# LeonOrou/OPF-Graph-Neural-Solver

Hardware: AMD Instinct MI355X
Metric: grids/sec (fwd+bwd) on batched case118, K=4 (higher is better)
Workload: dtype f32

## Files before the change

opf-graph-neural-solver_amd/csrc/gns_api.hip:

```cpp
#include <atomic>
#include <cmath>
#include <cstring>
#include <cstdlib>
#include <mutex>
#include "gns_kernels.h"
#include "gns_gridwg.h"

namespace {
struct GnsTuning {
  int fwd_mapping;
  int gw_pack;
  int fwd_waves;
  int fwd_plane;
  int dw_mfma;
  int train_mapping;
  int bwd_variant;
  int team;
  int bwds_mode;
  int bwds_chunks;
};
GnsTuning make_tuning() {
  GnsTuning t{0, 0, GNS_FWD_THREADS / 64, 2, 1, 0, 4, 0, 1, 0};
  if (const char* e = std::getenv("GNS_TEAM")) { const int v = std::atoi(e); if (v >= 0 && v <= GNS_MAX_TEAM) t.team = v; }
  if (const char* e = std::getenv("GNS_FWD_MAPPING")) t.fwd_mapping = !std::strcmp(e, "lane") ? 1 : (!std::strcmp(e, "lds") ? 2 : 0);
// ... 351 lines not shown
  *status = word ? 1 : 0;
  return GNS_OK;
}

extern "C" int gns_prepack_bytes(const gns_config* cfg, int64_t Bt, size_t* bytes) {
  int rc = check_cfg(cfg);
  if (rc != GNS_OK) return rc;
  if (!bytes || Bt <= 0) return GNS_EINVAL;
  const int64_t groups = (Bt + GNS_LANES - 1) / GNS_LANES;
  *bytes = (size_t)groups * gns_in_rows(cfg->n_bus, cfg->n_line) * GNS_LANES * 16;
  return GNS_OK;
}

extern "C" int gns_prepack(const gns_config* cfg, const void* topo_dev, const float* buses, const float* lines,
                           const float* generators, int64_t Bt, void* packed, size_t packed_bytes, void* stream) {
  size_t need = 0;
  int rc = gns_prepack_bytes(cfg, Bt, &need);
  if (rc != GNS_OK) return rc;
  if (!topo_dev || !buses || !lines || !generators || !packed) return GNS_EINVAL;
  if (packed_bytes < need) return GNS_ESIZE;
  return gns_launch_pack_inputs((const int*)topo_dev, buses, lines, generators, (float*)packed, cfg->n_bus, cfg->n_line, cfg->n_gen, Bt,
                                (Bt + GNS_LANES - 1) / GNS_LANES, (hipStream_t)stream);
}

static int lane_forward(const gns_config* cfg, const GnsFamilies& fam, const GnsFwdLayout& L, char* ws, float* pt, float* pin,
                        const int* topo_dev, const int* group_topo, const int* slot_grid, int64_t Bt, float* v, float* theta,
                        float* total_loss, float* last_loss, int save_state, hipStream_t st) {
  const int N = cfg->n_bus, E = cfg->n_line, K = cfg->K, d = cfg->latent_dim, h = cfg->hidden_dim;
  const GnsTuning& T = tuning();
  int rc;
  GnsFwdArgs A;
  std::memset(&A, 0, sizeof(A));
  A.topo = topo_dev; A.group_topo = group_topo; A.slot_grid = slot_grid; A.pt = pt; A.in = pin;
  A.state = (float*)(ws + L.off_state); A.lam = (float*)(ws + L.off_lam); A.msg = (float*)(ws + L.off_msg);
  A.v_out = v; A.theta_out = theta; A.total_out = total_loss; A.last_out = last_loss;
  for (int i = 0; i < fam.nfam; ++i) { A.t_off[i] = fam.t_off[i]; A.t_sz[i] = fam.t_sz[i]; }
  for (int k = 0; k < K; ++k) A.gw[k] = (float)std::pow((double)cfg->gamma, (double)(K - k));
  A.Bt = Bt; A.G = L.groups; A.N = N; A.E = E; A.K = K; A.save = save_state ? 1 : 0;
  const int team0 = lane_team(L.groups * GNS_LANES);
  A.team = team0;
  A.team_ws = (unsigned char*)(ws + L.off_team);
  int waves = T.fwd_waves;
  while (waves * A.team > GNS_MAXP) waves /= 2;
  A.part_idx = gns_part_index(waves * A.team);
  auto pick_planes = [&]() {
    A.plane = (device().fwd_ready && gns_fwd_plane_fits(N, A.team) && T.fwd_plane) ? 1 : 0;
    if (A.plane && gns_fwd_plane2_fits(N, A.team) && T.fwd_plane == 2) A.plane = 2;
  };
  pick_planes();
  if (A.team > 1) {
    const int per_cu = gns_fwd_blocks_per_cu(d, h, cfg->multiple_phi, A, waves * 64);
    if ((long long)per_cu * device().ncu < A.G * A.team) {
      A.team = 1;
      waves = T.fwd_waves;
      A.part_idx = gns_part_index(waves);
      pick_planes();
    }
  }
  if (team0 > 1 && hipMemsetAsync(A.team_ws, 0, (size_t)L.groups * GNS_TEAM_CTR_BYTES, st) != hipSuccess) return GNS_ELAUNCH;
  record_forward(1, waves, A.plane, A.team, -1);
  prof_mark(0, true, st);
  rc = gns_launch_forward(d, h, cfg->multiple_phi, A, waves * 64, st);
  prof_mark(0, false, st);
  return rc;
}

static int split_backward(const gns_config* cfg, const GnsFamilies& fam, const GnsFwdLayout& L, const GnsBwdsLayout& S, const char* fw,
                          char* bw, const int* topo_dev, const int* group_topo, const int* slot_grid, const float* params,
                          const void* packed_inputs, int64_t Bt, const float* grad_total, const float* grad_last, const float* grad_v,
                          const float* grad_theta, float* grad_params, hipStream_t st, const IgradOut* ig = nullptr) {
  const int N = cfg->n_bus, E = cfg->n_line, K = cfg->K, d = cfg->latent_dim, h = cfg->hidden_dim;
  int rc;
  GnsBwdsArgs A;
  std::memset(&A, 0, sizeof(A));
  A.topo = topo_dev; A.group_topo = group_topo; A.slot_grid = slot_grid;
  A.pt = (const float*)(fw + L.off_pt); A.pn = (const float*)(fw + L.off_pn);
  A.in = packed_inputs ? (const float*)packed_inputs : (const float*)(fw + L.off_in);
  A.state = (const float*)(fw + L.off_state); A.lam = (const float*)(fw + L.off_lam); A.msg = (const float*)(fw + L.off_msg);
  A.g_total = grad_total; A.g_last = grad_last; A.g_v = grad_v; A.g_theta = grad_theta;
  A.adj = (float*)(bw + S.off_adj); A.slots = (float*)(bw + S.off_slots); A.slab = (float*)(bw + S.off_slab);
  for (int i = 0; i < fam.nfam; ++i) {
    A.t_off[i] = fam.t_off[i]; A.t_sz[i] = fam.t_sz[i]; A.n_off[i] = fam.n_off[i]; A.n_sz[i] = fam.n_sz[i];
    A.g_off[i] = fam.g_off[i]; A.g_sz[i] = fam.g_sz[i];
  }
  A.Bt = Bt; A.G = S.groups; A.slab_floats = S.slab_floats; A.N = N; A.E = E; A.K = K;
  A.C = S.C; A.part_idx = gns_part_index(S.C); A.R = S.R;
  A.RB = (int)(1 + S.mq); A.RBA = (int)S.adj_rows;
  A.mode = cfg->multiple_phi ? tuning().bwds_mode : 2;
  const size_t lds = gns_bwds_phys_lds(N, &A.use_plane);
  if (ig) {
    A.igrad = ig->buf;
    if (hipMemsetAsync(A.igrad, 0, ig->bytes, st) != hipSuccess) return GNS_ELAUNCH;
  }
  record_backward(4, 1, A.mode, A.C, A.R, -1);
  prof_mark(1, true, st);
  for (int k = K - 1; k >= 0; --k) {
    A.k = k;
    A.gwk = (float)std::pow((double)cfg->gamma, (double)(K - k));
    rc = gns_launch_bwds_phys(A, lds, st);
    if (rc != GNS_OK) return rc;
    if (ig) {
      rc = gns_launch_bwds_igrad_phys(A, st);
      if (rc != GNS_OK) return rc;
    }
    rc = gns_launch_bwds_sweep(d, h, cfg->multiple_phi, A, st);
    if (rc != GNS_OK) return rc;
  }
  if (ig && (ig->buses || ig->lines || ig->gens)) {
    rc = gns_launch_bwds_igrad_unpack(A, ig->in_buses, ig->in_lines, ig->in_gens, cfg->n_gen, ig->buses, ig->lines, ig->gens, st);
    if (rc != GNS_OK) return rc;
  }
// ... 120 lines not shown
    rc = gns_gw_launch_backward(d, h, cfg->multiple_phi, G, GL.blocks, st);
    prof_mark(1, false, st);
    if (rc != GNS_OK) return rc;
    return gns_launch_reduce(G.slab, (float*)(bw + GL.off_part), (float*)(bw + GL.off_tmp), params, grad_params, GL.nslab,
                             GL.slab_floats, fam, K, d, h, st);
  }
  GnsFwdLayout L;
  gns_fwd_layout(N, E, d, h, K, cfg->multiple_phi, Bt, 1, &L);
  if (use_split_backward(cfg)) {
    GnsBwdsLayout S;
    gns_bwds_layout(N, E, d, h, K, cfg->multiple_phi, Bt, device().ncu, tuning().bwds_chunks, &S);
    if (fwd_workspace_bytes < L.total || bwd_workspace_bytes < S.total) return GNS_ESIZE;
    GnsFamilies fam; gns_families_padded(model->latent_dim, model->hidden_dim, d, h, K, cfg->multiple_phi, &fam);
    return split_backward(cfg, fam, L, S, (const char*)fwd_workspace, (char*)bwd_workspace, (const int*)topo_dev, nullptr, nullptr, params,
                          packed_inputs, Bt, grad_total, grad_last, grad_v, grad_theta, grad_params, (hipStream_t)stream);
  }
  GnsBwdLayout B;
  const int team = lane_team(Bt);
  gns_bwd_layout(N, E, d, h, K, cfg->multiple_phi, Bt, team, &B);
  if (fwd_workspace_bytes < L.total || bwd_workspace_bytes < B.total) return GNS_ESIZE;
  GnsFamilies fam; gns_families_padded(model->latent_dim, model->hidden_dim, d, h, K, cfg->multiple_phi, &fam);
  hipStream_t st = (hipStream_t)stream;
  const char* fw = (const char*)fwd_workspace;
  char* bw = (char*)bwd_workspace;
  const int blocks = (int)(B.groups * team < GNS_BWD_MAX_WG ? B.groups * team : GNS_BWD_MAX_WG);
  const long long nslab = (long long)blocks * GNS_BWD_WAVES;
  const bool v2 = tuning().dw_mfma && tuning().bwd_variant >= 2 && cfg->multiple_phi;
  if (!v2 && hipMemsetAsync(bw + B.off_slab, 0, (size_t)nslab * B.slab_floats * 4, st) != hipSuccess) return GNS_ELAUNCH;
  GnsBwdArgs A;
  std::memset(&A, 0, sizeof(A));
  A.topo = (const int*)topo_dev;
  A.pt = (const float*)(fw + L.off_pt); A.pn = (const float*)(fw + L.off_pn);
  A.in = packed_inputs ? (const float*)packed_inputs : (const float*)(fw + L.off_in);
  A.state = (const float*)(fw + L.off_state); A.lam = (const float*)(fw + L.off_lam); A.msg = (const float*)(fw + L.off_msg);
  A.g_total = grad_total; A.g_last = grad_last; A.g_v = grad_v; A.g_theta = grad_theta;
  A.adj = (float*)(bw + B.off_adj); A.slots = (float*)(bw + B.off_slots); A.slab = (float*)(bw + B.off_slab);
  for (int i = 0; i < fam.nfam; ++i) {
    A.t_off[i] = fam.t_off[i]; A.t_sz[i] = fam.t_sz[i]; A.n_off[i] = fam.n_off[i]; A.n_sz[i] = fam.n_sz[i];
    A.g_off[i] = fam.g_off[i]; A.g_sz[i] = fam.g_sz[i];
  }
  for (int k = 0; k < K; ++k) A.gw[k] = (float)std::pow((double)cfg->gamma, (double)(K - k));
  A.Bt = Bt; A.G = B.groups; A.slab_floats = B.slab_floats; A.N = N; A.E = E; A.K = K;
  A.part_idx = gns_part_index(GNS_BWD_WAVES * team);
  A.team = team; A.team_ws = (unsigned char*)(bw + B.off_team);
  if (team > 1 && hipMemsetAsync(A.team_ws, 0, (size_t)B.groups * GNS_TEAM_CTR_BYTES, st) != hipSuccess) return GNS_ELAUNCH;
  A.slab_dirty = v2 ? 1 : 0;
  record_backward(tuning().dw_mfma && cfg->multiple_phi && (tuning().bwd_variant == 2 || tuning().bwd_variant == 3) ? tuning().bwd_variant : 1,
                  tuning().dw_mfma, -1, -1, -1, -1);
  prof_mark(1, true, st);
  rc = gns_launch_backward(d, h, cfg->multiple_phi, tuning().dw_mfma, tuning().bwd_variant, A, blocks, st);
  prof_mark(1, false, st);
  if (rc != GNS_OK) return rc;
  return gns_launch_reduce(A.slab, (float*)(bw + B.off_part), (float*)(bw + B.off_tmp), params, grad_params, blocks, B.slab_floats,
                           fam, K, d, h, st, (long long)GNS_BWD_WAVES * B.slab_floats);
}

extern "C" int gns_backward_inputs(const gns_config* cfg, const void* topo_dev, const float* params,
                                   const float* buses, const float* lines, const float* generators, int64_t Bt, const void* packed_inputs,
                                   const void* fwd_workspace, size_t fwd_workspace_bytes, const float* grad_total,
                                   const float* grad_last, const float* grad_v, const float* grad_theta, float* grad_params,
                                   float* grad_buses, float* grad_lines, float* grad_generators,
                                   void* bwd_workspace, size_t bwd_workspace_bytes, void* stream) {
  int rc = check_cfg(cfg);
  if (rc != GNS_OK) return rc;
  if (!topo_dev || !params || !buses || !lines || !generators || !fwd_workspace || !bwd_workspace || Bt <= 0) return GNS_EINVAL;
  const gns_config* model = cfg; gns_config kcfg_;
  if (!kernel_config(model, &kcfg_) || cfg->K > GNS_MAX_K) return GNS_EUNSUPPORTED;
// ... 178 lines not shown
```

opf-graph-neural-solver_amd/csrc/gns_backward.hip:

```cpp
#include "gns_device.h"
#include "gns_kernels.h"

#include "gns_dw.h"

#ifndef GNS_BWD_PLANES
#define GNS_BWD_PLANES 1
#endif
typedef int gns_i8v __attribute__((ext_vector_type(8)));

template <int D, int H, bool MULTI, bool MFMA, int VAR>
__global__ void __launch_bounds__(GNS_BWD_THREADS) gns_backward_kernel(GnsBwdArgs A) {
  constexpr bool V2 = VAR >= 2;
  using C = GnsDims<D, H, MULTI>;
  constexpr int RB = C::RB;
  constexpr int W = GNS_BWD_WAVES;
  const int lane = threadIdx.x & 63;
  const int wave = __builtin_amdgcn_readfirstlane(threadIdx.x >> 6);
  const int N = A.N, E = A.E, K = A.K;
  cip topo = (cip)A.topo;
  cfp PT = (cfp)A.pt;
  cfp PN = (cfp)A.pn;
  const cip in_ptr = topo + topo[TH_IN_PTR], out_ptr = topo + topo[TH_OUT_PTR], is_gen = topo + topo[TH_IS_GEN],
            q2p = topo + topo[TH_Q2P], incd_ptr = topo + topo[TH_INCD_PTR],
            incd = topo + topo[TH_INCD], part = topo + topo[TH_PART] + A.part_idx * (GNS_MAXP + 1),
// ... 306 lines not shown
        cfp pnb = PN + A.n_off[fphi] + koff * A.n_sz[fphi];
        cfp ptb = PT + A.t_off[fphi] + koff * A.t_sz[fphi];
        f32x4 T1[NB1], T2, T4[NA4], TP1, TP2, TPm[NDM];
        const f32x4 z4 = {0.f, 0.f, 0.f, 0.f};
#pragma unroll
        for (int t = 0; t < NB1; ++t) T1[t] = z4;
#pragma unroll
        for (int t = 0; t < NA4; ++t) T4[t] = z4;
#pragma unroll
        for (int t = 0; t < NDM; ++t) TPm[t] = z4;
        T2 = z4; TP1 = z4; TP2 = z4;
        float ra[4], rb[4];
        const int rowmap = ((lane >> 5) & 1) + 4 * ((lane >> 4) & 1);
        const float* baseL = rec + rowmap * PL::RS + (lane & 15);
        const float* baseE = rec + rowmap * PE::RS + (lane & 15);
        const float* baseB = rec + rowmap * PB::RS + (lane & 15);
        auto accL = [&](auto ch_) -> f32x4& { constexpr int ch = decltype(ch_)::value; if constexpr (ch == 0) return T2; else return T1[ch - 1]; };
        auto accE = [&](auto ch_) -> f32x4& { constexpr int ch = decltype(ch_)::value; if constexpr (ch == 0) return TP1; else return TP2; };
        auto accB = [&](auto ch_) -> f32x4& { constexpr int ch = decltype(ch_)::value; return TPm[ch]; };
        auto putw = [&](int rs, int off, f2 v) { *reinterpret_cast<f2*>(rec + lane * rs + off) = v; };
        static_for<0, PB::RS / 2>([&](auto j_) { constexpr int j = decltype(j_)::value; putw(PB::RS, 2 * j, f2{0.f, 0.f}); });
        gws_w2r();
        for (int n = n0; n < n1; ++n) {
          const long long ar = adj_row(n), rr = state_row(k, n);
          const f4 a0 = *row_ptr(A.adj, ar, lane);
          f4 xsum = *row_ptr(A.adj, ar + 1, lane);
          const f4 s0 = *row_ptr(A.state, rr, lane);
          f2 xs[XL];
          f2 (&m)[D / 2] = reinterpret_cast<f2 (&)[D / 2]>(xs[2]);
          f2 (&S)[H / 2] = reinterpret_cast<f2 (&)[H / 2]>(xs[SOFF]);
          load_pairs<D>(A.state, rr + 1, lane, m);
          f2 macc[D / 2];
          load_pairs<D>(A.adj, ar + RM, lane, macc);
          load_pairs<H>(A.msg, ((((long long)k * A.G + g) * N + n) * C::NPHI + fphi) * C::HQ, lane, S);
          const int p0 = in_ptr[n], p1 = in_ptr[n + 1];
          xs[0] = f2{s0.x, s0.y}; xs[1] = f2{s0.z, s0.w};
          xs[XL - 1] = f2{(float)(p1 - p0), 1.f};
          f2 gS[H / 2];
          f2 a1[H / 2], a2[H / 2], g2[H / 2], g1[H / 2];
          {
            auto dr = gw_drain<PB, 0>(baseB, ra, rb, accB);
            dr.prologue();
            mlp2_fwd<LIN, H>(PT + A.t_off[C::NPHI + l] + koff * A.t_sz[C::NPHI + l], xs, a1, a2, dr);
            gws_r2w();
          }
          if constexpr (l == 2) {
            bwd_rows<OUTP, H>(nb, macc, g2);
          } else {
            const f2 g3s[1] = {f2{l == 0 ? a0.y : (is_gen[n] ? 0.f : a0.x), 0.f}};
            bwd_rows<2, H>(nb, g3s, g2);
          }
#pragma unroll
          for (int u = 0; u < H / 2; ++u) g2[u] = g2[u] * dlrelu2(a2[u]);
          static_for<0, H / 2>([&](auto j_) { constexpr int j = decltype(j_)::value; gws_putB(rec, lane, j, a2[j]); });
          gws_putB(rec, lane, H / 2, f2{1.f, 0.f});
          static_for<0, NA4>([&](auto t_) {
            constexpr int t = decltype(t_)::value;
            if constexpr (l == 2) {
              static_for<0, 6>([&](auto j_) { constexpr int j = decltype(j_)::value; if constexpr (6 * t + j < D / 2) gws_putA(rec, lane, j, macc[6 * t + j]); });
            } else {
              gws_putA(rec, lane, 0, f2{l == 0 ? a0.y : (is_gen[n] ? 0.f : a0.x), 0.f});
            }
            gws_w2r(); gws_pass(rec, lane, T4[t]); gws_r2w();
          });
          bwd_rows<H, H>(nb + NL::oW2, g2, g1);
#pragma unroll
          for (int u = 0; u < H / 2; ++u) g1[u] = g1[u] * dlrelu2(a1[u]);
// ... 134 lines not shown
        for (int t = 0; t < NB1; ++t) T1[t] = z4;
#pragma unroll
        for (int t = 0; t < NA4; ++t) T4[t] = z4;
#pragma unroll
        for (int t = 0; t < NDM; ++t) TPm[t] = z4;
        T2 = z4; TP1 = z4; TP2 = z4;
        cfp ptl = PT + A.t_off[C::NPHI + l] + koff * A.t_sz[C::NPHI + l];
        WFirst wf;
        using L0 = WLink<false, true>;
        using L1 = WLink<true, true>;
        using L2 = WLink<true, false>;
        SSTAMP(11)
        const bool first_family = (l == 2) || (l == 0 && k == K - 1);
        const bool step0 = k == 0;
        for (int n = n0; n < n1; ++n) {
          const long long ar = adj_row(n), rr = state_row(k, n);
          const f4 a0 = *row_ptr(A.adj, ar, lane);
          f4 xsum = f4{0.f, 0.f, 0.f, 0.f};
          const long long ar_ld = step0 ? adj_row(n0) : ar;
          if (!first_family) xsum = *row_ptr(A.adj, ar_ld + 1, lane);
          const f4 s0 = *row_ptr(A.state, rr, lane);
          f2 xs[XL];
          f2 (&m)[D / 2] = reinterpret_cast<f2 (&)[D / 2]>(xs[2]);
          f2 (&S)[H / 2] = reinterpret_cast<f2 (&)[H / 2]>(xs[SOFF]);
          load_pairs<D>(A.state, (step0 ? state_row(0, n0) : rr) + 1, lane, m);
          f2 macc[D / 2];
          if (l == 0 && k == K - 1) {
#pragma unroll
            for (int i = 0; i < D / 2; ++i) macc[i] = f2{0.f, 0.f};
          } else {
            load_pairs<D>(A.adj, (l != 2 ? ar_ld : ar) + RM, lane, macc);
          }
#ifdef GNS_ABLATE_HBM
          load_pairs<H>(A.msg, ((((long long)0 * A.G + g) * N + (n & 3)) * C::NPHI + fphi) * C::HQ, lane, S);
#else
          load_pairs<H>(A.msg, ((((long long)k * A.G + g) * N + n) * C::NPHI + fphi) * C::HQ, lane, S);
#endif
          const int p0 = in_ptr[n], p1 = in_ptr[n + 1];
          xs[0] = f2{s0.x, s0.y}; xs[1] = f2{s0.z, s0.w};
          xs[XL - 1] = f2{(float)(p1 - p0), 1.f};
          f2 gS[H / 2];
          SSTAMP(0)
          {
            f2 a1[H / 2], a2[H / 2], g2[H / 2], g1[H / 2];
            mlp2_fwd<LIN, H>(ptl, xs, a1, a2, NoBG{}, L0{nullptr, nb, &wf});
            SSTAMP(1)
            if constexpr (l == 2) {
              bwd_rows<OUTP, H>(nb, macc, g2, NoBG{}, L2{&wf, nullptr, nullptr});
            } else {
              const f2 g3s[1] = {f2{l == 0 ? a0.y : (is_gen[n] ? 0.f : a0.x), 0.f}};
              bwd_rows<2, H>(nb, g3s, g2, NoBG{}, std::conditional_t<FOLD4, L1, L2>{&wf, nb + NL::oW2, &wf});
            }
#pragma unroll
            for (int u = 0; u < H / 2; ++u) g2[u] = g2[u] * dlrelu2(a2[u]);
            if constexpr (FOLD4 || FOLDM) {
              static_for<0, H / 2>([&](auto j_) { constexpr int j = decltype(j_)::value; gws_putB<SW>(rec, lane, 8 + j, a2[j]); });
              gws_putB<SW>(rec, lane, 8 + H / 2, f2{1.f, 0.f});
              if constexpr (FOLDM) {
                static_for<0, 8>([&](auto j_) { constexpr int j = decltype(j_)::value; gws_putA<SW>(rec, lane, j, macc[j]); });
                gws_w2r(); gws_pass<SW, 16>(rec, lane, T4[0]); gws_r2w();
              }
            } else {
              static_for<0, H / 2>([&](auto j_) { constexpr int j = decltype(j_)::value; gws_putB<SW>(rec, lane, j, a2[j]); });
              gws_putB<SW>(rec, lane, H / 2, f2{1.f, 0.f});
              static_for<0, NA4>([&](auto t_) {
                constexpr int t = decltype(t_)::value;
                if constexpr (l == 2) {
                  static_for<0, 6>([&](auto j_) { constexpr int j = decltype(j_)::value; if constexpr (6 * t + j < D / 2) gws_putA<SW>(rec, lane, j, macc[6 * t + j]); });
                } else {
// ... 112 lines not shown
      });
      } else {
      static_for<0, 3>([&](auto o_) {
        constexpr int l = (decltype(o_)::value == 0) ? 2 : decltype(o_)::value - 1;
        constexpr int fphi = MULTI ? (l == 0 ? 1 : (l == 1 ? 0 : 2)) : 0;
        constexpr int OUT = (l == 2) ? D : 1, OUTP = OUT + (OUT & 1);
        if (l == 2 && k == K - 1) return;
        LEngine<C::LF_IN, H, OUT, OUTP, MFMA> engL;
        PEngine<C::PHI_IN, H, MFMA> engP;
        engL.init(lane); engP.init(lane);
        for (int n = n0; n < n1; ++n) {
          const long long ar = adj_row(n), rr = state_row(k, n);
          const f4 a0 = *row_ptr(A.adj, ar, lane);
          f4 xsum = *row_ptr(A.adj, ar + 1, lane);
          const f4 s0 = *row_ptr(A.state, rr, lane);
          f2 m[D / 2];
          load_pairs<D>(A.state, rr + 1, lane, m);
          constexpr int XL = (C::LF_IN + 1) / 2;
          f2 gx[XL];
          f2 (&macc)[D / 2] = reinterpret_cast<f2 (&)[D / 2]>(gx[2]);
          f2 (&gS)[H / 2] = reinterpret_cast<f2 (&)[H / 2]>(gx[2 + D / 2]);
          gx[0] = f2{0.f, 0.f}; gx[1] = f2{0.f, 0.f}; gx[XL - 1] = f2{0.f, 0.f};
          load_pairs<D>(A.adj, ar + RM, lane, macc);
          if constexpr (MULTI) {
#pragma unroll
            for (int j = 0; j < H / 2; ++j) gS[j] = f2{0.f, 0.f};
          } else {
            load_pairs<H>(A.adj, ar + 2, lane, gS);
          }
          const int p0 = in_ptr[n], p1 = in_ptr[n + 1];
          {
            f2 x[XL];
            f2 (&S)[H / 2] = reinterpret_cast<f2 (&)[H / 2]>(x[2 + D / 2]);
            load_pairs<H>(A.msg, ((((long long)k * A.G + g) * N + n) * C::NPHI + fphi) * C::HQ, lane, S);
            x[0] = f2{s0.x, s0.y}; x[1] = f2{s0.z, s0.w};
#pragma unroll
            for (int i = 0; i < D / 2; ++i) x[2 + i] = m[i];
            x[XL - 1] = f2{(float)(p1 - p0), 0.f};
            f2 a1[H / 2], a2[H / 2], g3[OUTP / 2], g2[H / 2], g1[H / 2];
            mlp2_fwd<C::LF_IN, H>(PT + A.t_off[C::NPHI + l] + koff * A.t_sz[C::NPHI + l], x, a1, a2);
            if constexpr (l == 0) g3[0] = f2{a0.y, 0.f};
            else if constexpr (l == 1) g3[0] = f2{is_gen[n] ? 0.f : a0.x, 0.f};
            else {
#pragma unroll
              for (int j = 0; j < D / 2; ++j) g3[j] = macc[j];
            }
            mlp_bwd<C::LF_IN, H, OUTP, 2 * XL, true>(PN + A.n_off[C::NPHI + l] + koff * A.n_sz[C::NPHI + l], a1, a2, g3, g2, g1, gx);
            xsum.x += gx[0].x; xsum.y += gx[0].y; xsum.z += gx[1].x;
            engL.accumulate(rec, lane, x, a1, a2, g1, g2, g3);
          }
          if constexpr (MULTI) {
            if (p0 < p1) load_pairs<D>(A.state, rr + 1, lane, m);
#ifdef GNS_ABLATE_MSGBWD
            for (int p = p0; p < p0; ++p) {
#else
            for (int p = p0; p < p1; ++p) {
#endif
              f2 xe[(C::PHI_IN + 1) / 2], a1[H / 2], a2[H / 2], g2[H / 2], g1[H / 2];
              edge_input(p, m, xe);
              mlp2_fwd<C::PHI_IN, H>(PT + A.t_off[fphi] + koff * A.t_sz[fphi], xe, a1, a2);
              mlp2_bwd<C::PHI_IN, H, D, true>(PN + A.n_off[fphi] + koff * A.n_sz[fphi], a1, a2, gS, g2, g1, macc);
              engP.accumulate(rec, lane, xe, a1, g1, g2);
            }
          } else {
            store_pairs<H>(A.adj, ar + 2, lane, gS);
          }
          *row_ptr(A.adj, ar + 1, lane) = xsum;
// ... 172 lines not shown
```

opf-graph-neural-solver_amd/csrc/gns_backward_split.hip:

```cpp
#include "gns_device.h"
#include "gns_kernels.h"
#include "gns_dw.h"

typedef int gns_i8v __attribute__((ext_vector_type(8)));
#ifndef GNS_BWDS_ONE_LAYOUT
#define GNS_BWDS_ONE_LAYOUT 0
#endif
#ifndef GNS_BWDS_WPE
#define GNS_BWDS_WPE 2
#endif
#ifndef GNS_BWDS_KEEP_SLOPES
#define GNS_BWDS_KEEP_SLOPES 1
#endif
#if GNS_BWDS_KEEP_SLOPES
#define GNS_SLOPES(sl) sl
#define GNS_SLOPE_OF(sl, layer, act, u) sl[layer][u]
#else
#define GNS_SLOPES(sl) nullptr
#define GNS_SLOPE_OF(sl, layer, act, u) dlrelu2(act[u])
#endif
#ifndef GNS_BWDS_FRESH_INPUTS
#define GNS_BWDS_FRESH_INPUTS 1
#endif
#define GNS_BWDS_PHYS_THREADS (GNS_BWDS_PHYS_WAVES * 64)
// ... 243 lines not shown
  using L0 = typename B::L0; using L1 = typename B::L1; using L2 = typename B::L2;
  static constexpr int LIN = B::LIN, XL = B::XL, SOFF = B::SOFF, NB1 = B::NB1, XT = B::XT, W2OFF = B::W2OFF;
  static constexpr bool WIDE = B::WIDE;
  static constexpr int fphi = MULTI ? (l == 0 ? 1 : (l == 1 ? 0 : 2)) : 0;
  static constexpr int OUT = (l == 2) ? D : 1, OUTP = OUT + (OUT & 1), NA4 = (OUTP + 11) / 12;
  using NL = NLay<LIN, H, OUTP>;
  static constexpr bool FOLD4 = WIDE && l < 2 && XT + H + 1 <= 16;
  static constexpr bool FOLDM = GwSubWide::NA >= 16 && WIDE && l == 2 && XT + H + 1 <= 16 && H + (OUT - 16) <= 16;

  static constexpr int NT4 = FOLD4 ? 1 : (FOLDM ? 1 : NA4);
  f32x4 T1[NB1], T2, T4[NT4];
  cfp nb, ptl;

  __device__ __forceinline__ void init(const GnsBwdsArgs& A) {
    const long long koff = A.k;
    nb = (cfp)A.pn + A.n_off[C::NPHI + l] + koff * A.n_sz[C::NPHI + l];
    ptl = (cfp)A.pt + A.t_off[C::NPHI + l] + koff * A.t_sz[C::NPHI + l];
    scalar_cache_warm(ptl, A.t_sz[C::NPHI + l]);
#if !GNS_BWDS_ONE_LAYOUT
    scalar_cache_warm(nb, A.n_sz[C::NPHI + l]);
#endif
    const f32x4 z4 = {0.f, 0.f, 0.f, 0.f};
#pragma unroll
    for (int t = 0; t < NB1; ++t) T1[t] = z4;
#pragma unroll
    for (int t = 0; t < NT4; ++t) T4[t] = z4;
    T2 = z4;
  }

  template <bool ACC_GS, bool STEP0, bool IG = false>
  __device__ __forceinline__ void bus(const GnsBwdsArgs& A, float* rec, int lane, long long g, int n, float g3s, f2 (&xs)[XL],
                                      f2 (&macc)[D / 2], f4& xsum, f2 (&gS)[H / 2]) {
    f2 (&S)[H / 2] = reinterpret_cast<f2 (&)[H / 2]>(xs[SOFF]);
    load_pairs<H>(A.msg, ((((long long)A.k * A.G + g) * A.N + n) * C::NPHI + fphi) * C::HQ, lane, S);
    WFirst wf;
    f2 a1[H / 2], a2[H / 2], g2[H / 2], g1[H / 2];
    f2 sl[2][H / 2];
    using TL [[maybe_unused]] = TLay<LIN, H, OUTP>;
#if GNS_BWDS_ONE_LAYOUT
    (void)wf;
    mlp2_fwd<LIN, H>(ptl, xs, a1, a2, NoBG{}, NoLink{}, GNS_SLOPES(sl));
#else
    using LKm = std::conditional_t<STEP0, NoLink, L2>; using LKs = std::conditional_t<STEP0, std::conditional_t<FOLD4, L0, NoLink>, std::conditional_t<FOLD4, L1, L2>>;
    if constexpr (STEP0) {
      f2 u4[H / 2];
      const f2 (&st)[2] = reinterpret_cast<const f2 (&)[2]>(xs[0]);
      const f2 (&tl)[(LIN - 4 - D + 1) / 2] = reinterpret_cast<const f2 (&)[(LIN - 4 - D + 1) / 2]>(xs[SOFF]);
      phi_head<4, H>(ptl, st, u4);
      phi_tail<LIN, H, 4 + D>(ptl, u4, tl, a1, a2, NoBG{}, NoLink{}, GNS_SLOPES(sl));
    } else {
      mlp2_fwd<LIN, H>(ptl, xs, a1, a2, NoBG{}, L0{nullptr, nb, &wf}, GNS_SLOPES(sl));
    }
#endif
#if GNS_BWDS_ONE_LAYOUT
    if constexpr (l == 2) {
      bwd_rows_fwd_layout<H, OUTP>(ptl + TL::oW4, macc, g2);
    } else {
      const f2 g3v[1] = {f2{g3s, 0.f}};
      bwd_rows_fwd_layout<H, 2>(ptl + TL::oW4, g3v, g2);
    }
#else
    if constexpr (l == 2) {
      bwd_rows<OUTP, H>(nb, macc, g2, NoBG{}, LKm{&wf, nullptr, nullptr});
    } else {
      const f2 g3v[1] = {f2{g3s, 0.f}};
      bwd_rows<2, H>(nb, g3v, g2, NoBG{}, LKs{&wf, nb + NL::oW2, &wf});
    }
// ... 592 lines not shown
```

opf-graph-neural-solver_amd/csrc/gns_common.h:

```cpp
#pragma once
#include <stdint.h>
#include <stddef.h>

#if defined(__HIPCC__)
#include <hip/hip_runtime.h>
#define GNS_HD __host__ __device__
#else
#define GNS_HD
#endif

#define GNS_LANES 64
#define GNS_TOPO_MAGIC 0x474e5332
#define GNS_NPART 8
#define GNS_MAXW 16
#define GNS_MAXP 32
#define GNS_MAX_TEAM 4

enum {
  TH_MAGIC = 0, TH_N, TH_E, TH_GN,
  TH_IN_PTR,
  TH_IN_EID,
  TH_IN_SRC,
  TH_IN_A,
  TH_IN_B,
// ... 69 lines not shown
  int outk[6];
};

static inline void gns_families_padded(int dr, int hr, int dk, int hk, int K, int multi, GnsFamilies* f) {
  f->nfam = multi ? 6 : 4;
  f->nphi = multi ? 3 : 1;
  f->dr = dr; f->hr = hr; f->dk = dk; f->hk = hk;
  int64_t fo = 0, to = 0, no = 0, go = 0;
  for (int i = 0; i < f->nfam; ++i) {
    bool is_phi = i < f->nphi;
    const bool wide_out = is_phi ? multi != 0 : i == f->nfam - 1;
    f->in[i] = is_phi ? dr + 5 : 4 + 2 * dr;
    f->out[i] = wide_out ? dr : 1;
    f->outk[i] = wide_out ? dk : 1;
    const int ink = is_phi ? dk + 5 : 4 + 2 * dk;
    f->phi_of[i] = is_phi ? -1 : (multi ? (i == 3 ? 1 : (i == 4 ? 0 : 2)) : 0);
    f->flat_sz[i] = gns_flat_block(f->in[i], hr, f->out[i]);
    f->t_sz[i] = gns_t_block(is_phi, dk, hk, f->outk[i]);
    f->n_sz[i] = gns_n_block(is_phi, dk, hk, f->outk[i]);
    f->g_sz[i] = is_phi ? (int64_t)ink * hk + hk + (int64_t)hk * hk + hk
                        : (int64_t)gns_lin(dk, hk) * hk + hk + (int64_t)hk * hk + hk + (int64_t)f->outk[i] * hk + f->outk[i];
    f->flat_off[i] = fo; f->t_off[i] = to; f->n_off[i] = no; f->g_off[i] = go;
    fo += f->flat_sz[i] * K; to += f->t_sz[i] * K; no += f->n_sz[i] * K; go += f->g_sz[i] * K;
  }
  f->flat_total = fo; f->g_total = go; f->t_total = to + 64; f->n_total = no + 64;
}
static inline void gns_families(int d, int h, int K, int multi, GnsFamilies* f) { gns_families_padded(d, h, d, h, K, multi, f); }

struct GnsFwdLayout {
  int64_t groups;
  int64_t mq;
  int64_t rows_bus;
  int64_t slots;
  size_t off_pt, off_pn, off_in, off_lam, off_state, off_msg, off_team, total;
};
#define GNS_TEAM_MAX_GROUPS 128

static inline size_t gns_align256(size_t x) { return (x + 255) & ~(size_t)255; }

static inline void gns_fwd_layout(int N, int E, int d, int h, int K, int multi, int64_t Bt, int save, GnsFwdLayout* L) {
  GnsFamilies f; gns_families(d, h, K, multi, &f);
  L->groups = (Bt + GNS_LANES - 1) / GNS_LANES;
  L->mq = (d + 3) / 4;
  L->rows_bus = 1 + L->mq;
  L->slots = save ? K + 1 : 2;
  size_t o = 0;
  L->off_pt = o;    o = gns_align256(o + (size_t)f.t_total * 4);
  L->off_pn = o;    o = gns_align256(o + (size_t)f.n_total * 4);
  L->off_in = o;    o = gns_align256(o + (size_t)L->groups * gns_in_rows(N, E) * GNS_LANES * 16);
  L->off_lam = o;   o = gns_align256(o + (size_t)K * L->groups * GNS_LANES * 8);
  L->off_state = o; o = gns_align256(o + (size_t)L->slots * L->groups * N * L->rows_bus * GNS_LANES * 16);
  L->off_msg = o;   o = gns_align256(o + (save ? (size_t)K * L->groups * N * (multi ? 3 : 1) * ((h + 3) / 4) * GNS_LANES * 16 : 0));
  L->off_team = o;  o = gns_align256(o + (L->groups <= GNS_TEAM_MAX_GROUPS ? gns_team_bytes(L->groups) : 0));
  L->total = o;
}

#define GNS_BWD_WAVES 8
#define GNS_RED_PARTS 64
struct GnsBwdLayout {
  int64_t groups, mq, rows_bus;
  int64_t slab_floats;
  int64_t adj_rows;
  int64_t nslab;
  size_t off_adj, off_slots, off_slab, off_part, off_tmp, off_team, total;
};
#define GNS_BWD_MAX_WG 256

static inline void gns_bwd_layout(int N, int E, int d, int h, int K, int multi, int64_t Bt, int team, GnsBwdLayout* B) {
  GnsFamilies f; gns_families(d, h, K, multi, &f);
  B->groups = (Bt + GNS_LANES - 1) / GNS_LANES;
  B->mq = (d + 3) / 4;
  B->rows_bus = 1 + B->mq;
  B->slab_floats = (f.g_total + 63) / 64 * 64;
  B->adj_rows = B->rows_bus + 1 + (multi ? 0 : (h + 3) / 4);
  int64_t wg = B->groups * team < GNS_BWD_MAX_WG ? B->groups * team : GNS_BWD_MAX_WG;
  B->nslab = wg * GNS_BWD_WAVES;
  size_t o = 0;
  B->off_adj = o;   o = gns_align256(o + (size_t)B->groups * N * B->adj_rows * GNS_LANES * 16);
  B->off_slots = o; o = gns_align256(o + (size_t)B->groups * 6 * E * GNS_LANES * 4);
  B->off_slab = o;  o = gns_align256(o + (size_t)B->nslab * B->slab_floats * 4);
  B->off_part = o;  o = gns_align256(o + (size_t)GNS_RED_PARTS * B->slab_floats * 4);
  B->off_tmp = o;   o = gns_align256(o + (size_t)B->slab_floats * 4);
  B->off_team = o;  o = gns_align256(o + (team > 1 ? gns_team_bytes(B->groups) : 0));
  B->total = o;
}
// ... 35 lines not shown
```

opf-graph-neural-solver_amd/csrc/gns_device.h:

```cpp
#pragma once
#include <hip/hip_runtime.h>
#include <type_traits>
#include "gns_common.h"

typedef float f2 __attribute__((ext_vector_type(2)));
typedef float f4 __attribute__((ext_vector_type(4)));
typedef float f16v __attribute__((ext_vector_type(16)));
typedef const __attribute__((address_space(4))) float* cfp;
typedef const __attribute__((address_space(4))) int* cip;

__device__ __forceinline__ bool gns_group_topo(const int* set, const int* group_topo, long long g, int N, int E, cip& topo) {
  topo = (cip)set + ((cip)group_topo)[g];
  return topo[TH_MAGIC] == GNS_TOPO_MAGIC && topo[TH_N] == N && topo[TH_E] == E;
}
typedef const __attribute__((address_space(4))) f16v* cf16p;
typedef f16v f16u __attribute__((aligned(4)));
typedef const __attribute__((address_space(4))) f16u* cf16up;

struct GnsTeam {
  unsigned* ctr;
  float* red;
  int size, member;
  unsigned epoch;
  int* failed;
// ... 452 lines not shown
}

__device__ __forceinline__ f4* row_ptr_lanewise(float* base, long long row, int lane) {
  return reinterpret_cast<f4*>(base) + row * GNS_LANES + lane;
}

template <int D>
__device__ __forceinline__ void load_pairs(const float* base, long long row, int lane, f2 (&m)[D / 2]) {
  static_for<0, (D + 3) / 4>([&](auto q_) {
    constexpr int q = decltype(q_)::value;
    const f4 t = *row_ptr(base, row + q, lane);
    m[2 * q] = f2{t.x, t.y};
    if constexpr (2 * q + 1 < D / 2) m[2 * q + 1] = f2{t.z, t.w};
  });
}
template <int D>
__device__ __forceinline__ void store_pairs_nt(float* base, long long row, int lane, const f2 (&m)[D / 2]) {
  static_for<0, (D + 3) / 4>([&](auto q_) {
    constexpr int q = decltype(q_)::value;
    f4 t = {m[2 * q].x, m[2 * q].y, 0.f, 0.f};
    if constexpr (2 * q + 1 < D / 2) { t.z = m[2 * q + 1].x; t.w = m[2 * q + 1].y; }
    __builtin_nontemporal_store(t, row_ptr(base, row + q, lane));
  });
}
template <int D>
__device__ __forceinline__ void store_pairs(float* base, long long row, int lane, const f2 (&m)[D / 2]) {
  static_for<0, (D + 3) / 4>([&](auto q_) {
    constexpr int q = decltype(q_)::value;
    f4 t = {m[2 * q].x, m[2 * q].y, 0.f, 0.f};
    if constexpr (2 * q + 1 < D / 2) { t.z = m[2 * q + 1].x; t.w = m[2 * q + 1].y; }
    *row_ptr(base, row + q, lane) = t;
  });
}
```

opf-graph-neural-solver_amd/csrc/gns_forward.hip:

```cpp
#include "gns_device.h"
#ifndef GNS_FWD_GEN_SKIP
#define GNS_FWD_GEN_SKIP 1
#endif
#include "gns_kernels.h"

__global__ void gns_pack_params_kernel(const float* __restrict__ flat, float* __restrict__ pt, float* __restrict__ pn,
                                       GnsFamilies fam, int K, int D, int H) {
  const int blk = blockIdx.x;
  const int f = blk / K, k = blk % K;
  const bool is_phi = f < fam.nphi;
  const int Dr = fam.dr, Hr = fam.hr;
  const int INr = fam.in[f], OUTr = fam.out[f];
  const int OUT = fam.outk[f], OUTP = OUT + (OUT & 1);
  const float* src = flat + fam.flat_off[f] + (int64_t)k * fam.flat_sz[f];
  const int sW1 = 0, sb1 = INr * Hr, sW2 = sb1 + Hr, sb2 = sW2 + Hr * Hr, sW4 = sb2 + Hr, sb4 = sW4 + OUTr * Hr;
  auto W2r = [&](int j, int i) -> float { return (j < Hr && i < Hr) ? src[sW2 + j * Hr + i] : 0.f; };
  auto b1r = [&](int j) -> float { return j < Hr ? src[sb1 + j] : 0.f; };
  auto b2r = [&](int j) -> float { return j < Hr ? src[sb2 + j] : 0.f; };
  float* t = pt + fam.t_off[f] + (int64_t)k * fam.t_sz[f];
  float* n = pn + fam.n_off[f] + (int64_t)k * fam.n_sz[f];
  if (is_phi) {
    const int IN = D + 5, INP = IN + (IN & 1);
    auto W1r = [&](int j, int i) -> float {
      if (j >= Hr) return 0.f;
// ... 231 lines not shown
  float tot_part = 0.f, last_part = 0.f;
  const float invN = 1.0f / (float)N;

#ifdef GNS_STAMPS
  long long tph[6] = {0, 0, 0, 0, 0, 0};
  long long tlast = clock64();
#define FSTAMP(i) { const long long tn = clock64(); tph[i] += tn - tlast; tlast = tn; }
#else
#define FSTAMP(i)
#endif
  for (int k = 0; k < K; ++k) {
    const int rs = A.save ? k : (k & 1), ws = A.save ? k + 1 : ((k + 1) & 1);
    FSTAMP(5)
    const long long koff = (long long)k;
    auto update_unit = [&](auto grp_, int n) {
      constexpr int grp = decltype(grp_)::value;
      constexpr int NL = grp == 0 ? 2 : 1, L0 = grp == 0 ? 0 : 2;
      const long long rr = state_row(rs, n), wr = state_row(ws, n);
      const f4 s0 = *row_ptr(A.state, rr, lane);
      f2 m[D / 2];
      if (k == 0) {
#pragma unroll
        for (int i = 0; i < D / 2; ++i) m[i] = f2{0.f, 0.f};
      } else {
        load_pairs<D>(A.state, rr + 1, lane, m);
      }
      const int p0 = in_ptr[n], p1 = in_ptr[n + 1];
      f2 S[NL][H / 2];
#pragma unroll
      for (int j = 0; j < NL; ++j)
#pragma unroll
        for (int q = 0; q < H / 2; ++q) S[j][q] = f2{0.f, 0.f};
      constexpr int NF = MULTI ? NL : 1;
#if GNS_FWD_GEN_SKIP
      const bool skip_v = grp == 0 && is_gen[n] != 0;
#else
      const bool skip_v = false;
#endif
      f2 uh[NF][H / 2];
      if (p0 < p1) {
        static_for<0, NF>([&](auto j_) {
          constexpr int j = decltype(j_)::value;
          constexpr int l = L0 + j;
          constexpr int fphi = MULTI ? (l == 0 ? 1 : (l == 1 ? 0 : 2)) : 0;
          if (MULTI && l == 1 && skip_v) return;
          phi_head<D, H>(PT + A.t_off[fphi] + koff * A.t_sz[fphi], m, uh[j]);
        });
      }
      for (int p = p0; p < p1; ++p) {
        const f4 e0 = *row_ptr(IN, row_ein + 3LL * p, lane), e1 = *row_ptr(IN, row_ein + 3LL * p + 1, lane);
        const f2 xt[3] = {f2{e0.x, e0.y}, f2{e0.z, e0.w}, f2{e1.x, 0.f}};
        static_for<0, NF>([&](auto j_) {
          constexpr int j = decltype(j_)::value;
          constexpr int l = L0 + j;
          constexpr int fphi = MULTI ? (l == 0 ? 1 : (l == 1 ? 0 : 2)) : 0;
          if (MULTI && l == 1 && skip_v) return;
          f2 a1[H / 2], a2[H / 2];
          phi_tail<C::PHI_IN, H, D>(PT + A.t_off[fphi] + koff * A.t_sz[fphi], uh[j], xt, a1, a2);
#pragma unroll
          for (int q = 0; q < H / 2; ++q) S[j][q] += a2[q];
        });
      }
      f2 vth_new = f2{s0.x, s0.y};
      static_for<0, NL>([&](auto j_) {
        constexpr int j = decltype(j_)::value;
        constexpr int l = L0 + j;
        constexpr int fphi = MULTI ? (l == 0 ? 1 : (l == 1 ? 0 : 2)) : 0;
        constexpr int js = MULTI ? j : 0;
#ifndef GNS_ABLATE_MSG_SAVE
        if (A.save && (MULTI || l == 0))
#else
        if (false)
#endif
          store_pairs_nt<H>(A.msg, ((((long long)k * A.G + g) * N + n) * C::NPHI + fphi) * C::HQ, lane, S[js]);
        if (l == 1 && skip_v) {
          vth_new.x = s0.x;
          if (!(use_plane && tsize == 1) || GNS_FWD_ROW_STORES) reinterpret_cast<float*>(row_ptr(A.state, wr, lane))[0] = s0.x;
          return;
        }
        f2 x[(C::LF_IN + 1) / 2];
        x[0] = f2{s0.x, s0.y}; x[1] = f2{s0.z, s0.w};
#pragma unroll
        for (int i = 0; i < D / 2; ++i) x[2 + i] = m[i];
#pragma unroll
        for (int q = 0; q < H / 2; ++q) x[2 + D / 2 + q] = S[js][q];
        x[2 + D / 2 + H / 2] = f2{(float)(p1 - p0), 0.f};
        f2 a1[H / 2], a2[H / 2];
        if constexpr (l < 2) {
          f2 y[1];
          mlp_fwd<C::LF_IN, H, 2>(PT + A.t_off[C::NPHI + l] + koff * A.t_sz[C::NPHI + l], x, a1, a2, y);
          float* r0 = reinterpret_cast<float*>(row_ptr(A.state, wr, lane));
          const bool row_needed = !(use_plane && tsize == 1) || GNS_FWD_ROW_STORES;
          if constexpr (l == 0) { vth_new.y = s0.y + y[0].x; if (row_needed) r0[1] = vth_new.y; }
          else { vth_new.x = is_gen[n] ? s0.x : s0.x + y[0].x; if (row_needed) r0[0] = vth_new.x; }
        } else {
          f2 upd_m[D / 2], m_new[D / 2];
          mlp_fwd<C::LF_IN, H, D>(PT + A.t_off[C::NPHI + 2] + koff * A.t_sz[C::NPHI + 2], x, a1, a2, upd_m);
#pragma unroll
          for (int i = 0; i < D / 2; ++i) m_new[i] = m[i] + upd_m[i];
          if (k < K - 1) store_pairs_nt<D>(A.state, wr + 1, lane, m_new);
        }
      });
      if constexpr (grp == 0) { if (use_plane) plane[n * GNS_LANES + lane] = vth_new; }
    };
    const bool draw = A.save == 0 && tsize == 1;
    const bool last_step = k == K - 1 && GNS_FWD_SKIP_LAST_M;
    const int ub = last_step ? n0 : u0, ue = last_step ? n1 : u1, uall = last_step ? N : 2 * N;
// ... 219 lines not shown
```

opf-graph-neural-solver_amd/csrc/gns_kernels.h:

```cpp
#pragma once
#include <hip/hip_runtime.h>
#include "../../include/gns_hip.h"
#include "gns_common.h"

#define GNS_FWD_THREADS 1024
#define GNS_FWD_MAX_THREADS 1024
#define GNS_BWD_THREADS 512
#define GNS_MAX_K 64
#define GNS_FWD_RED_BYTES (2 * GNS_MAXW * GNS_LANES * 2 * 4)
#define GNS_FWD_DYN_LDS_MAX (160 * 1024 - 64)
static inline int gns_fwd_plane_fits(int N, int team) {
  return (size_t)N * GNS_LANES * 8 + (team == 1 ? GNS_FWD_RED_BYTES : 0) <= (size_t)GNS_FWD_DYN_LDS_MAX;
}
static inline int gns_fwd_plane2_fits(int N, int team) {
  return team == 1 && 2 * (size_t)N * GNS_LANES * 8 + GNS_FWD_RED_BYTES <= (size_t)GNS_FWD_DYN_LDS_MAX;
}

#define GNS_FOR_EACH_DIMS(X) X(20, 14) X(20, 10) X(10, 10)
#define GNS_FOR_EACH_DIMS_PERSISTENT(X) X(20, 10) X(10, 10)
#define GNS_FOR_EACH_DIMS_GWB(X) X(20, 10) X(10, 10)

template <int D, int H, bool MULTI>
struct GnsDims {
  static constexpr int NPHI = MULTI ? 3 : 1;
  static constexpr int PHI_IN = D + 5;
  static constexpr int PHI_OUT = MULTI ? D : 1;
  static constexpr int PHI_OUTP = PHI_OUT + (PHI_OUT & 1);
  static constexpr int L_IN = 4 + 2 * D;
  static constexpr int LF_IN = 4 + D + H + 1;
  static constexpr int HQ = (H + 3) / 4;
  static constexpr int MQ = (D + 3) / 4;
  static constexpr int RB = 1 + MQ;
};

struct GnsFwdArgs {
  const int* topo;
  const float* pt;
  const float* in;
  float* state;
  float* lam;
  float* msg;
  float* v_out; float* theta_out; float* total_out; float* last_out;
  long long t_off[6], t_sz[6];
  float gw[GNS_MAX_K];
  long long Bt, G;
  int N, E, K, save, part_idx;
  int plane;
  int team;
  unsigned char* team_ws;
  const int* group_topo;
  const int* slot_grid;
};

struct GnsBwdArgs {
  const int* topo;
  const float* pt; const float* pn;
  const float* in;
  const float* state;
  const float* lam;
  const float* msg;
  const float* g_total; const float* g_last; const float* g_v; const float* g_theta;
  float* adj;
  float* slots;
  float* slab;
  long long t_off[6], t_sz[6], n_off[6], n_sz[6], g_off[6], g_sz[6];
  float gw[GNS_MAX_K];
  long long Bt, G, slab_floats;
  int N, E, K, part_idx;
  int team; unsigned char* team_ws;
  int slab_dirty;
};

int gns_launch_backward(int d, int h, int multi, int mfma, int variant, const GnsBwdArgs& A, int blocks, hipStream_t st);
int gns_backward_persistent_supported(int d, int h);
int gns_launch_reduce(const float* slab, float* part, float* tmp, const float* flat, float* grad, long long nslab, long long sf,
                      const GnsFamilies& fam, int K, int D, int H, hipStream_t st, long long stride = 0);
int gns_launch_forward(int d, int h, int multi, const GnsFwdArgs& A, int threads, hipStream_t st);
int gns_fwd_init_device();
int gns_fwd_blocks_per_cu(int d, int h, int multi, const GnsFwdArgs& A, int threads);
int gns_launch_pack_params(const float* flat, float* pt, float* pn, const GnsFamilies& fam, int K, int D, int H, hipStream_t st);
int gns_launch_pack_inputs(const int* topo, const float* buses, const float* lines, const float* gens, float* out, int N,
                           int E, int Gn, long long Bt, long long groups, hipStream_t st,
                           const int* group_topo = nullptr, const int* slot_grid = nullptr);

struct GnsBwdsArgs {
  const int* topo;
  const float* pt; const float* pn;
  const float* in; const float* state; const float* lam; const float* msg;
  const float* g_total; const float* g_last; const float* g_v; const float* g_theta;
  float* adj; float* slots; float* slab;
  long long t_off[6], t_sz[6], n_off[6], n_sz[6], g_off[6], g_sz[6];
  long long Bt, G, slab_floats;
  float gwk;
  int N, E, K, k;
  int C, part_idx, R;
  int RB, RBA;
  int use_plane;
  int mode;
  const int* group_topo;
  const int* slot_grid;
  float* igrad;
};
int gns_bwds_supported(int d, int h, int multi);
size_t gns_bwds_phys_lds(int N, int* use_plane);
int gns_launch_bwds_phys(const GnsBwdsArgs& A, size_t lds, hipStream_t st);
int gns_launch_bwds_sweep(int d, int h, int multi, const GnsBwdsArgs& A, hipStream_t st);
int gns_launch_bwds_igrad_phys(const GnsBwdsArgs& A, hipStream_t st);
int gns_launch_bwds_igrad_unpack(const GnsBwdsArgs& A, const float* buses, const float* lines, const float* gens, int Gn,
                                 float* grad_buses, float* grad_lines, float* grad_gens, hipStream_t st);
int gns_bwds_init_device();
```

Baseline: 6.022 million.

## Split saved hidden sums into float4 rows plus float2 plane; skip gen-bus saves

Saved message hidden sums (H=10) used to be padded to HQ float4 rows, so every row wasted 8 bytes. They are now stored as H/4 float4 rows plus one separate float2 plane, which cuts the save and reload traffic between forward and backward. The forward pass also skips saving the l==1 phi sums for generator buses, and the backward substitutes zeros for them on the assumption that those values are unused there. This adds a new workspace region and pointer plumbing, and it relies on H%4==2 (enforced by static_assert) and on the zero substitution being correct.

```diff
diff --git a/opf-graph-neural-solver_amd/csrc/gns_api.hip b/opf-graph-neural-solver_amd/csrc/gns_api.hip
--- a/opf-graph-neural-solver_amd/csrc/gns_api.hip
+++ b/opf-graph-neural-solver_amd/csrc/gns_api.hip
@@ -407,7 +407,7 @@
   GnsFwdArgs A;
   std::memset(&A, 0, sizeof(A));
   A.topo = topo_dev; A.group_topo = group_topo; A.slot_grid = slot_grid; A.pt = pt; A.in = pin;
-  A.state = (float*)(ws + L.off_state); A.lam = (float*)(ws + L.off_lam); A.msg = (float*)(ws + L.off_msg);
+  A.state = (float*)(ws + L.off_state); A.lam = (float*)(ws + L.off_lam); A.msg = (float*)(ws + L.off_msg); A.msg2 = (float*)(ws + L.off_msg2);
   A.v_out = v; A.theta_out = theta; A.total_out = total_loss; A.last_out = last_loss;
   for (int i = 0; i < fam.nfam; ++i) { A.t_off[i] = fam.t_off[i]; A.t_sz[i] = fam.t_sz[i]; }
   for (int k = 0; k < K; ++k) A.gw[k] = (float)std::pow((double)cfg->gamma, (double)(K - k));
@@ -451,7 +451,7 @@
   A.topo = topo_dev; A.group_topo = group_topo; A.slot_grid = slot_grid;
   A.pt = (const float*)(fw + L.off_pt); A.pn = (const float*)(fw + L.off_pn);
   A.in = packed_inputs ? (const float*)packed_inputs : (const float*)(fw + L.off_in);
-  A.state = (const float*)(fw + L.off_state); A.lam = (const float*)(fw + L.off_lam); A.msg = (const float*)(fw + L.off_msg);
+  A.state = (const float*)(fw + L.off_state); A.lam = (const float*)(fw + L.off_lam); A.msg = (const float*)(fw + L.off_msg); A.msg2 = (const float*)(fw + L.off_msg2);
   A.g_total = grad_total; A.g_last = grad_last; A.g_v = grad_v; A.g_theta = grad_theta;
   A.adj = (float*)(bw + S.off_adj); A.slots = (float*)(bw + S.off_slots); A.slab = (float*)(bw + S.off_slab);
   for (int i = 0; i < fam.nfam; ++i) {
@@ -638,7 +638,7 @@
   A.topo = (const int*)topo_dev;
   A.pt = (const float*)(fw + L.off_pt); A.pn = (const float*)(fw + L.off_pn);
   A.in = packed_inputs ? (const float*)packed_inputs : (const float*)(fw + L.off_in);
-  A.state = (const float*)(fw + L.off_state); A.lam = (const float*)(fw + L.off_lam); A.msg = (const float*)(fw + L.off_msg);
+  A.state = (const float*)(fw + L.off_state); A.lam = (const float*)(fw + L.off_lam); A.msg = (const float*)(fw + L.off_msg); A.msg2 = (const float*)(fw + L.off_msg2);
   A.g_total = grad_total; A.g_last = grad_last; A.g_v = grad_v; A.g_theta = grad_theta;
   A.adj = (float*)(bw + B.off_adj); A.slots = (float*)(bw + B.off_slots); A.slab = (float*)(bw + B.off_slab);
   for (int i = 0; i < fam.nfam; ++i) {
diff --git a/opf-graph-neural-solver_amd/csrc/gns_backward.hip b/opf-graph-neural-solver_amd/csrc/gns_backward.hip
--- a/opf-graph-neural-solver_amd/csrc/gns_backward.hip
+++ b/opf-graph-neural-solver_amd/csrc/gns_backward.hip
@@ -362,7 +362,7 @@
           load_pairs<D>(A.state, rr + 1, lane, m);
           f2 macc[D / 2];
           load_pairs<D>(A.adj, ar + RM, lane, macc);
-          load_pairs<H>(A.msg, ((((long long)k * A.G + g) * N + n) * C::NPHI + fphi) * C::HQ, lane, S);
+          load_pairs_split_or_zero<H>(A.msg, A.msg2, (((long long)k * A.G + g) * N + n) * C::NPHI + fphi, lane, MULTI && l == 1 && is_gen[n], S);
           const int p0 = in_ptr[n], p1 = in_ptr[n + 1];
           xs[0] = f2{s0.x, s0.y}; xs[1] = f2{s0.z, s0.w};
           xs[XL - 1] = f2{(float)(p1 - p0), 1.f};
@@ -563,9 +563,9 @@
             load_pairs<D>(A.adj, (l != 2 ? ar_ld : ar) + RM, lane, macc);
           }
 #ifdef GNS_ABLATE_HBM
-          load_pairs<H>(A.msg, ((((long long)0 * A.G + g) * N + (n & 3)) * C::NPHI + fphi) * C::HQ, lane, S);
+          load_pairs_split<H>(A.msg, A.msg2, (((long long)0 * A.G + g) * N + (n & 3)) * C::NPHI + fphi, lane, S);
 #else
-          load_pairs<H>(A.msg, ((((long long)k * A.G + g) * N + n) * C::NPHI + fphi) * C::HQ, lane, S);
+          load_pairs_split_or_zero<H>(A.msg, A.msg2, (((long long)k * A.G + g) * N + n) * C::NPHI + fphi, lane, MULTI && l == 1 && is_gen[n], S);
 #endif
           const int p0 = in_ptr[n], p1 = in_ptr[n + 1];
           xs[0] = f2{s0.x, s0.y}; xs[1] = f2{s0.z, s0.w};
@@ -744,7 +744,7 @@
           {
             f2 x[XL];
             f2 (&S)[H / 2] = reinterpret_cast<f2 (&)[H / 2]>(x[2 + D / 2]);
-            load_pairs<H>(A.msg, ((((long long)k * A.G + g) * N + n) * C::NPHI + fphi) * C::HQ, lane, S);
+            load_pairs_split_or_zero<H>(A.msg, A.msg2, (((long long)k * A.G + g) * N + n) * C::NPHI + fphi, lane, MULTI && l == 1 && is_gen[n], S);
             x[0] = f2{s0.x, s0.y}; x[1] = f2{s0.z, s0.w};
 #pragma unroll
             for (int i = 0; i < D / 2; ++i) x[2 + i] = m[i];
diff --git a/opf-graph-neural-solver_amd/csrc/gns_backward_split.hip b/opf-graph-neural-solver_amd/csrc/gns_backward_split.hip
--- a/opf-graph-neural-solver_amd/csrc/gns_backward_split.hip
+++ b/opf-graph-neural-solver_amd/csrc/gns_backward_split.hip
@@ -299,7 +299,7 @@
   __device__ __forceinline__ void bus(const GnsBwdsArgs& A, float* rec, int lane, long long g, int n, float g3s, f2 (&xs)[XL],
                                       f2 (&macc)[D / 2], f4& xsum, f2 (&gS)[H / 2]) {
     f2 (&S)[H / 2] = reinterpret_cast<f2 (&)[H / 2]>(xs[SOFF]);
-    load_pairs<H>(A.msg, ((((long long)A.k * A.G + g) * A.N + n) * C::NPHI + fphi) * C::HQ, lane, S);
+    load_pairs_split<H>(A.msg, A.msg2, (((long long)A.k * A.G + g) * A.N + n) * C::NPHI + fphi, lane, S);
     WFirst wf;
     f2 a1[H / 2], a2[H / 2], g2[H / 2], g1[H / 2];
     f2 sl[2][H / 2];
diff --git a/opf-graph-neural-solver_amd/csrc/gns_common.h b/opf-graph-neural-solver_amd/csrc/gns_common.h
--- a/opf-graph-neural-solver_amd/csrc/gns_common.h
+++ b/opf-graph-neural-solver_amd/csrc/gns_common.h
@@ -125,7 +125,7 @@
   int64_t mq;
   int64_t rows_bus;
   int64_t slots;
-  size_t off_pt, off_pn, off_in, off_lam, off_state, off_msg, off_team, total;
+  size_t off_pt, off_pn, off_in, off_lam, off_state, off_msg, off_msg2, off_team, total;
 };
 #define GNS_TEAM_MAX_GROUPS 128
 
@@ -143,7 +143,9 @@
   L->off_in = o;    o = gns_align256(o + (size_t)L->groups * gns_in_rows(N, E) * GNS_LANES * 16);
   L->off_lam = o;   o = gns_align256(o + (size_t)K * L->groups * GNS_LANES * 8);
   L->off_state = o; o = gns_align256(o + (size_t)L->slots * L->groups * N * L->rows_bus * GNS_LANES * 16);
-  L->off_msg = o;   o = gns_align256(o + (save ? (size_t)K * L->groups * N * (multi ? 3 : 1) * ((h + 3) / 4) * GNS_LANES * 16 : 0));
+  const size_t hsum_rows = save ? (size_t)K * L->groups * N * (multi ? 3 : 1) : 0;
+  L->off_msg = o;   o = gns_align256(o + hsum_rows * (h / 4) * GNS_LANES * 16);
+  L->off_msg2 = o;  o = gns_align256(o + hsum_rows * GNS_LANES * 8);
   L->off_team = o;  o = gns_align256(o + (L->groups <= GNS_TEAM_MAX_GROUPS ? gns_team_bytes(L->groups) : 0));
   L->total = o;
 }
diff --git a/opf-graph-neural-solver_amd/csrc/gns_device.h b/opf-graph-neural-solver_amd/csrc/gns_device.h
--- a/opf-graph-neural-solver_amd/csrc/gns_device.h
+++ b/opf-graph-neural-solver_amd/csrc/gns_device.h
@@ -508,3 +508,41 @@
     *row_ptr(base, row + q, lane) = t;
   });
 }
+
+__device__ __forceinline__ const f2* row_ptr2(const float* base, long long row, int lane) {
+  return reinterpret_cast<const f2*>(base) + row * GNS_LANES + lane;
+}
+__device__ __forceinline__ f2* row_ptr2(float* base, long long row, int lane) {
+  return reinterpret_cast<f2*>(base) + row * GNS_LANES + lane;
+}
+template <int D>
+__device__ __forceinline__ void load_pairs_split(const float* base4, const float* base2, long long r, int lane, f2 (&m)[D / 2]) {
+  static_assert(D % 4 == 2, "split form: D/4 float4 rows + one float2");
+  static_for<0, D / 4>([&](auto q_) {
+    constexpr int q = decltype(q_)::value;
+    const f4 t = *row_ptr(base4, r * (D / 4) + q, lane);
+    m[2 * q] = f2{t.x, t.y};
+    m[2 * q + 1] = f2{t.z, t.w};
+  });
+  m[D / 2 - 1] = *row_ptr2(base2, r, lane);
+}
+template <int D>
+__device__ __forceinline__ void store_pairs_split_nt(float* base4, float* base2, long long r, int lane, const f2 (&m)[D / 2]) {
+  static_assert(D % 4 == 2, "split form: D/4 float4 rows + one float2");
+  static_for<0, D / 4>([&](auto q_) {
+    constexpr int q = decltype(q_)::value;
+    const f4 t = {m[2 * q].x, m[2 * q].y, m[2 * q + 1].x, m[2 * q + 1].y};
+    __builtin_nontemporal_store(t, row_ptr(base4, r * (D / 4) + q, lane));
+  });
+  __builtin_nontemporal_store(m[D / 2 - 1], row_ptr2(base2, r, lane));
+}
+template <int D>
+__device__ __forceinline__ void load_pairs_split_or_zero(const float* base4, const float* base2, long long r, int lane, bool zero,
+                                                         f2 (&m)[D / 2]) {
+  if (zero) {
+#pragma unroll
+    for (int i = 0; i < D / 2; ++i) m[i] = f2{0.f, 0.f};
+  } else {
+    load_pairs_split<D>(base4, base2, r, lane, m);
+  }
+}
diff --git a/opf-graph-neural-solver_amd/csrc/gns_forward.hip b/opf-graph-neural-solver_amd/csrc/gns_forward.hip
--- a/opf-graph-neural-solver_amd/csrc/gns_forward.hip
+++ b/opf-graph-neural-solver_amd/csrc/gns_forward.hip
@@ -287,8 +287,9 @@
 #pragma unroll
         for (int q = 0; q < H / 2; ++q) S[j][q] = f2{0.f, 0.f};
       constexpr int NF = MULTI ? NL : 1;
+      const bool gen_bus = grp == 0 && is_gen[n] != 0;
 #if GNS_FWD_GEN_SKIP
-      const bool skip_v = grp == 0 && is_gen[n] != 0;
+      const bool skip_v = gen_bus;
 #else
       const bool skip_v = false;
 #endif
@@ -323,11 +324,11 @@
         constexpr int fphi = MULTI ? (l == 0 ? 1 : (l == 1 ? 0 : 2)) : 0;
         constexpr int js = MULTI ? j : 0;
 #ifndef GNS_ABLATE_MSG_SAVE
-        if (A.save && (MULTI || l == 0))
+        if (A.save && (MULTI ? !(l == 1 && gen_bus) : l == 0))
 #else
         if (false)
 #endif
-          store_pairs_nt<H>(A.msg, ((((long long)k * A.G + g) * N + n) * C::NPHI + fphi) * C::HQ, lane, S[js]);
+          store_pairs_split_nt<H>(A.msg, A.msg2, (((long long)k * A.G + g) * N + n) * C::NPHI + fphi, lane, S[js]);
         if (l == 1 && skip_v) {
           vth_new.x = s0.x;
           if (!(use_plane && tsize == 1) || GNS_FWD_ROW_STORES) reinterpret_cast<float*>(row_ptr(A.state, wr, lane))[0] = s0.x;
diff --git a/opf-graph-neural-solver_amd/csrc/gns_kernels.h b/opf-graph-neural-solver_amd/csrc/gns_kernels.h
--- a/opf-graph-neural-solver_amd/csrc/gns_kernels.h
+++ b/opf-graph-neural-solver_amd/csrc/gns_kernels.h
@@ -29,6 +29,8 @@
   static constexpr int L_IN = 4 + 2 * D;
   static constexpr int LF_IN = 4 + D + H + 1;
   static constexpr int HQ = (H + 3) / 4;
+  static constexpr int HQ4 = H / 4;
+  static_assert(H % 4 == 2, "the saved hidden sums are h/4 float4 rows + one float2 plane (gns_common.h, gns_fwd_layout)");
   static constexpr int MQ = (D + 3) / 4;
   static constexpr int RB = 1 + MQ;
 };
@@ -40,6 +42,7 @@
   float* state;
   float* lam;
   float* msg;
+  float* msg2;
   float* v_out; float* theta_out; float* total_out; float* last_out;
   long long t_off[6], t_sz[6];
   float gw[GNS_MAX_K];
@@ -59,6 +62,7 @@
   const float* state;
   const float* lam;
   const float* msg;
+  const float* msg2;
   const float* g_total; const float* g_last; const float* g_v; const float* g_theta;
   float* adj;
   float* slots;
@@ -86,7 +90,7 @@
 struct GnsBwdsArgs {
   const int* topo;
   const float* pt; const float* pn;
-  const float* in; const float* state; const float* lam; const float* msg;
+  const float* in; const float* state; const float* lam; const float* msg; const float* msg2;
   const float* g_total; const float* g_last; const float* g_v; const float* g_theta;
   float* adj; float* slots; float* slab;
   long long t_off[6], t_sz[6], n_off[6], n_sz[6], g_off[6], g_sz[6];
```

Result: faster. 6.082 million (median of 6 runs) (+1.0%).
